# panuelosj/polystokes

Hardware: AMD Instinct MI355X
Metric: Stokes-solve wall ms/step (assembly+PCG) on 256^3 grid; CG iters/sec (lower is better)
Workload: dtype f64; 1 GPU; synthetic lid-driven cavity 256x256x256, reduced tiles (tile=16, pad=2), jacobi-PCG, tol 1e-3; parallelism=1 GPU

## Files before the change

polystokes_amd/__init__.py:

```python
import ctypes as C
import os
import subprocess

import numpy as np

from . import _abi
from ._abi import (FieldsIn, FieldsOut, Params, Scene, Stats, default_params)

_HERE = os.path.dirname(os.path.abspath(__file__))
LIB_PATH = os.environ.get("PS_LIB") or os.path.join(_HERE, "libpolystokes_hip.so")
_lib = None

EXPORTED_SYMBOLS = [
    "ps_abi_version", "ps_reduced_dof", "ps_context_create", "ps_context_destroy", "ps_last_error", "ps_params_default",
    "ps_upload_fields", "ps_step_device", "ps_setup_device", "ps_solve_device", "ps_download_fields",
    "polystokes_step", "ps_apply_operator", "ps_apply_preconditioner", "ps_query_array", "ps_read_array",
    "ps_export_component_matrices", "ps_export_matrices", "ps_export_stats", "ps_bench_kernel", "ps_memory_stats", "ps_set_interrupt", "ps_solve_exported_system",
    "ps_set_slab", "ps_set_brick", "ps_comm_unique_id", "ps_comm_init_rccl", "ps_comm_selftest", "ps_comm_init_tcp", "ps_dist_stats",
    "ps_group_create", "ps_group_destroy", "ps_group_rank", "ps_group_step",
    "ps_set_warm_start", "ps_download_solution_fields", "ps_upload_density_field", "ps_set_surface_tension",
    "ps_set_solid_boundary", "ps_set_rheology", "ps_set_solve_precision",
    "ps_upload_fields_device", "ps_upload_density_field_device", "ps_download_fields_device", "ps_download_solution_fields_device",
    "ps_step_device_fields", "ps_set_velocity_extrapolation",
]
# ... 162 lines not shown
    fi = FieldsIn()
    fi.nx, fi.ny, fi.nz = fields.nx, fields.ny, fields.nz
    fi.dx, fi.dt = fields.dx, fields.dt
    fi.orig[0] = fi.orig[1] = fi.orig[2] = 0.0
    fi.density = fields.density
    cv = getattr(fields, "collisionvel", None)
    for a in range(3):
        fi.vel[a] = device_address(fields.vel[a])
        fi.collisionvel[a] = device_address(cv[a]) if cv is not None else None
    fi.surface, fi.collision, fi.viscosity = (device_address(fields.surface), device_address(fields.collision),
                                              device_address(fields.viscosity))
    w = getattr(fields, "weights", None)
    for i in range(14):
        fi.weights[i] = device_address(w[i]) if w is not None else None
    return fi


_DT = {(1, "i"): np.int8, (4, "i"): np.int32, (4, "f"): np.float32, (8, "f"): np.float64, (4, "u"): np.uint32}


def _kind(name):
    if name.endswith(("Labels", "Indices", ".col", ".ptr", "Region", "Perm", ".chunkInfo", ".chunkRep", ".code")) or name.startswith("faceRow"):
        return "i"
    if name in ("valuesCoded", "columns16", "diagonalsCoded", "fusedStep", "streamRuns", "rowPerLane", "chebInner32", "warmStartUsed", "densityField", "launchWalk",
                "surfaceTensionReducedFaces", "solidBoundary", "solidSlipEdges", "rheologyModel", "rheologyIterations",
                "solvePrecisionUsed", "solvePassIterations",
                "velocityExtrapolation", "extrapolationLayerX", "extrapolationLayerY", "extrapolationLayerZ", "extrapolationCounts"):
        return "i"
    if name in ("ownedX", "ownedY", "ownedZ"):
        return "f"
    if False:
        return "i"
    if name == "reducedRowFace":
        return "u"
    return "f"


def process_memory_stats():
    v = (C.c_int64 * 4)()
    lib().ps_memory_stats(None, v)
    return {"live_bytes": int(v[0]), "peak_bytes": int(v[1]), "contexts": int(v[3])}


class PolyStokesError(RuntimeError):
    pass


# ... 392 lines not shown
```

polystokes_amd/csrc/ps_blocks.hip:

```cpp
#include "ps_context.hpp"
#include "ps_setup_util.hpp"

using namespace ps;

namespace {

constexpr int BS = SETUP_BS;

struct BlockArgs {
    Grid g;
    double invDx;
    const float* lw[7];
    const float* fw[7];
    const int32_t* lab[7];
    const int32_t* act[7];
    const int32_t* reg[7];
    const int32_t* sys[7];
    const int32_t* sysT[3];
    const int32_t* faceRow[3];
    const float* vel[3];
    const float* cvel[3];
    CellField visc;
    FaceDensity dens;
    int64_t nP, nA, faceOff[3];
// ... 922 lines not shown
            hipLaunchKernelGGL(k_St_edges<true>, dim3(gridFor(ne, BS)), dim3(BS), 0, stream, A, e, (int32_t*)nullptr, St.ptr.p, St.col.p,
                               v, St.code.p, rhsPT.p, uInv.p, wantExport ? uDiag.p : (double*)nullptr);
        }
    };
    {
        const int64_t n = g.count(0);
        hipLaunchKernelGGL(k_St_cells<false>, dim3(gridFor(n, BS)), dim3(BS), 0, stream, A, St.ptr.p, (const int32_t*)nullptr,
                           (int32_t*)nullptr, (double*)nullptr, (int8_t*)nullptr, (double*)nullptr, (double*)nullptr, (double*)nullptr);
        for (int e = 0; e < 3; ++e) {
            const int64_t ne = g.count(4 + e);
            hipLaunchKernelGGL(k_St_edges<false>, dim3(gridFor(ne, BS)), dim3(BS), 0, stream, A, e, St.ptr.p, (const int32_t*)nullptr,
                               (int32_t*)nullptr, (double*)nullptr, (int8_t*)nullptr, (double*)nullptr, (double*)nullptr, (double*)nullptr);
        }
        St.nnz = exclusiveScanI32(St.ptr.p, nSystem + 1);
        if (St.nnz != S.nnz) throw Error("internal: nnz(S^T) != nnz(S)");
        St.col.alloc((size_t)St.nnz); St.code.alloc((size_t)St.nnz);
        fillSt(forceFp64Values);
    }
    {
        const bool ok = readCounter(CTR_CODE_FAIL) == 0;
        if (!ok && !forceFp64Values) { fillS(true); fillSt(true); }
        S.packed = St.packed = ok && !forceFp64Values;
        valuesCodedHost = S.packed ? 1 : 0;
        buildDiagonalCodes();
        buildStreams(true);
        columns16Host = (S.col16ok ? 1 : 0) | (St.col16ok ? 2 : 0);
    }
}
```

polystokes_amd/csrc/ps_context.hip:

```cpp
#include <algorithm>
#include <chrono>
#include <cstdio>
#include <cstring>
#include <ctime>
#include <fstream>

#include "ps_context.hpp"
#include "ps_setup_util.hpp"

using namespace ps;

namespace {

struct StageTimer {
    hipEvent_t ev[PS_STAGE_COUNT + 1];
    hipStream_t s;
    int n = 0;
    explicit StageTimer(hipStream_t st) : s(st) {
        for (auto& e : ev) HIP_CHECK(hipEventCreate(&e));
    }
    ~StageTimer() { for (auto& e : ev) (void)hipEventDestroy(e); }
    void mark(int i) { HIP_CHECK(hipEventRecord(ev[i], s)); }
    double ms(int a, int b) { float f = 0; HIP_CHECK(hipEventElapsedTime(&f, ev[a], ev[b])); return f; }
};
// ... 195 lines not shown
        T.mark(1);
        classifyCells();
        if (P.doReducedRegions) constructReducedRegions(); else constructOnlyActiveRegions();
        setupPhaseDone = 0;
        return;
    }
    if (phase == 1) {
        classifyFaces();
        classifyEdges();
        T.mark(2);
        if (P.doReducedRegions) constructCenterReducedIndices(0);
        setupPhaseDone = 1;
        return;
    }
    if (P.doReducedRegions) {
        constructCenterReducedIndices(1);
        constructFacesReducedIndices();
        constructEdgesReducedIndices();
    }
    T.mark(3);
    constructActiveIndices();
    computeRheology();
    T.mark(4);
    if (P.doReducedRegions) {
        computeCenterOfMasses();
        computeLeastSquaresFits();
        computeReducedMassMatrices();
        computeReducedViscosityMatricesInteriorOnly();
    } else {
        fbItems = 0;
    }
    T.mark(5);
    constructMatrixBlocks();
    T.mark(6);
    assembleSystemPressureStressFactored();
    constructGuessVectors();
    T.mark(7);
    constructPreconditioner();
    T.mark(8);
    HIP_CHECK(hipStreamSynchronize(stream));
    const auto w1 = std::chrono::high_resolution_clock::now();
    std::memset(&lastStats, 0, sizeof(lastStats));
    lastStats.result = PS_INCOMPLETE;
    fillDimData(&lastStats);
    lastStats.solveData[0] = -1; lastStats.solveData[1] = -1; lastStats.solveData[2] = -1; lastStats.solveData[3] = -1;
    lastStats.solveData[4] = 1000.0 * (double)(std::clock() - Z.c0) / CLOCKS_PER_SEC;
    lastStats.solveData[5] = std::chrono::duration<double, std::milli>(w1 - Z.w0).count();
    lastStats.stage_ms[PS_STAGE_WEIGHTS] = T.ms(0, 1);
    lastStats.stage_ms[PS_STAGE_CLASSIFY] = T.ms(1, 2);
    lastStats.stage_ms[PS_STAGE_REGIONS] = T.ms(2, 3);
    lastStats.stage_ms[PS_STAGE_INDICES] = T.ms(3, 4);
    lastStats.stage_ms[PS_STAGE_TILE_MATRICES] = T.ms(4, 5);
    lastStats.stage_ms[PS_STAGE_BLOCKS] = T.ms(5, 6);
    lastStats.stage_ms[PS_STAGE_ASSEMBLE] = T.ms(6, 7);
    lastStats.stage_ms[PS_STAGE_PRECOND] = T.ms(7, 8);
    setupState.reset();
    setupPhaseDone = 2;
// ... 102 lines not shown
    regHost("solidBoundary", &solidBoundaryUsed, 1, 4);
    if (solidBoundaryUsed == PS_SOLID_FREE_SLIP) reg("solidSlipEdges", slipEdges.p, 1, 4);
    regHost("rheologyModel", &rheoModelUsed, 1, 4);
    if (rheoModelUsed != PS_RHEOLOGY_NEWTONIAN) {
        reg("rheologyStrainRate", rheoRate.p, g.count(0), 4);
        reg("rheologyViscosity", rheoMu.p, g.count(0), 4);
        regHost("rheologyIterations", rheoIters.data(), (int64_t)rheoIters.size(), 4);
    }
    regHost("velocityExtrapolation", &extrapUsedHost, 1, 4);
    if (extrapUsedHost > 0) {
        static const char* axn[3] = {"X", "Y", "Z"};
        for (int a = 0; a < 3; ++a) reg(std::string("extrapolationLayer") + axn[a], extrapLayer[a].p, g.count(1 + a), 1);
        reg("extrapolationCounts", extrapCounts.p, extrapUsedHost, 4);
    }
    if (P.preconditioner == PS_PRE_DIAGONAL) regp("dinv", dinv.p, nSystem, permSys.p, 0);
    if (isSolved) {
        regp("recoveredActiveVelocity", recovered.p, nActiveVs, permRow.p, 0);
        reg("recoveredReducedVelocity", recovered.p ? recovered.p + nActiveVs : nullptr, nReducedVs, 8);
    }
    regHost("valuesCoded", &valuesCodedHost, 1, 4);
    diagFlagsHost = (uCoded ? 1 : 0) | (mcCoded ? 2 : 0);
    regHost("diagonalsCoded", &diagFlagsHost, 1, 4);
    regHost("columns16", &columns16Host, 1, 4);
    regHost("fusedStep", &fusedStepHost, 1, 4);
    regHost("launchWalk", launchWalkHost, 5 * LAUNCH_WALK_FIELDS, 4);
    chebInner32Host = chebInner32 ? 1 : 0;
    regHost("chebInner32", &chebInner32Host, 1, 4);
    streamRunsHost[0] = S.col16ok ? (int32_t)S.uniqueLen : 0; streamRunsHost[1] = S.col16ok ? (int32_t)S.streamLen : 0;
    streamRunsHost[2] = St.col16ok ? (int32_t)St.uniqueLen : 0; streamRunsHost[3] = St.col16ok ? (int32_t)St.streamLen : 0;
    regHost("streamRuns", streamRunsHost, 4, 4);
    rowPerLaneHost[0] = ((S.ellok && S.packed) ? 1 : 0) | ((St.ellok && St.packed) ? 2 : 0); rowPerLaneHost[1] = ilPlaneMajor;
    regHost("rowPerLane", rowPerLaneHost, 2, 4);
    reg("sysPerm", permSys.p, nSystem, 4);
    reg("rowPerm", permRow.p, nActiveVs, 4);
    reg("S.ptr", S.ptr.p, S.rows + 1, 4); reg("S.col", S.col.p, S.nnz, 4); reg("S.val", S.val.p, S.nnz, 8);
    reg("St.ptr", St.ptr.p, St.rows + 1, 4); reg("St.col", St.col.p, St.nnz, 4); reg("St.val", St.val.p, St.nnz, 8);
    if (S.col16ok) { reg("S.chunkInfo", S.chunkInfo.p, (int64_t)S.nChunks * 4, 4); reg("S.chunkRep", S.chunkRep.p, S.nChunks, 4); }
    if (St.col16ok) { reg("St.chunkInfo", St.chunkInfo.p, (int64_t)St.nChunks * 4, 4); reg("St.chunkRep", St.chunkRep.p, St.nChunks, 4); }
    if (S.packed) reg("S.code", S.code.p, S.nnz, 1);
    if (St.packed) reg("St.code", St.code.p, St.nnz, 1);
    reg("reducedRowFace", rrowFace.p, nReducedRows, 4);
    reg("reducedRowRegion", rrowRegion.p, nReducedRows, 4);
    static const char* ax[3] = {"X", "Y", "Z"};
    for (int a = 0; a < 3; ++a) {
        reg(std::string("vel") + ax[a], velOut[a].p, g.count(1 + a), 4);
        reg(std::string("valid") + ax[a], valid[a].p, g.count(1 + a), 4);
// ... 138 lines not shown
int32_t ps_reduced_dof(void) { return PS_RD; }

ps_context* ps_context_create(int32_t device) {
    int count = 0;
    hipError_t e = hipGetDeviceCount(&count);
    if (e != hipSuccess || count <= 0) {
        g_createError = "polystokes: no HIP device available (the product path has no CPU fallback)";
        std::fprintf(stderr, "%s\n", g_createError.c_str());
        return nullptr;
    }
    if (device < 0 || device >= count) {
        g_createError = "polystokes: device index out of range";
        std::fprintf(stderr, "%s\n", g_createError.c_str());
        return nullptr;
    }
    ps_context* c = new ps_context();
    c->device = device;
    if (hipSetDevice(device) != hipSuccess || hipStreamCreateWithFlags(&c->stream, hipStreamNonBlocking) != hipSuccess) {
        delete c;
        g_createError = "polystokes: cannot initialise HIP device";
        std::fprintf(stderr, "%s\n", g_createError.c_str());
        return nullptr;
    }
    ps_params_default(&c->P);
    return c;
}

void ps_context_destroy(ps_context* c) {
    if (!c) return;
    (void)hipSetDevice(c->device);
    (void)hipStreamSynchronize(c->stream);
    ps_dist_release(c);
    hipStream_t s = c->ownsStream ? c->stream : nullptr;
    if (c->pinnedCounters) (void)hipHostFree(c->pinnedCounters);
    if (c->pinnedScan) (void)hipHostFree(c->pinnedScan);
    for (auto& e : c->fieldEv) if (e) (void)hipEventDestroy(e);
    delete c;
    ps::releaseDeferred(ps::orphanFrees());
    if (s) (void)hipStreamDestroy(s);
}

const char* ps_last_error(const ps_context* c) { return c ? c->err.c_str() : g_createError.c_str(); }

void ps_params_default(ps_params* p) {
    std::memset(p, 0, sizeof(*p));
    p->mindensity = 1; p->maxdensity = 100000;
    p->matrixSetup = PS_PRESSURE_STRESS; p->solverType = PS_PCG_MATRIX_VECTOR_PRODUCTS;
    p->doSolve = 1; p->keepNonConvergedResults = 1; p->useWarmStart = 1;
    p->tolerance = 1e-3; p->maxSolverIterations = 5000;
    p->useInputSurfaceWeights = 1; p->useInputCollisionWeights = 1;
    p->activeLiquidBoundaryLayerSize = 2; p->activeSolidBoundaryLayerSize = 2;
    p->doReducedRegions = 1; p->doTile = 1; p->tileSize = 16; p->tilePadding = 2;
    p->preconditioner = PS_PRE_IDENTITY; p->indexOrder = PS_ORDER_VOXEL_TILES; p->negateCollision = 1;
}

int32_t ps_upload_fields(ps_context* c, const ps_params* p, const ps_fields_in* in) {
    if (!c) return PS_FAILED;
    PS_TRY(c, { c->upload(p, in); return PS_SUCCESS; })
}
// ... 599 lines not shown
```

polystokes_amd/csrc/ps_context.hpp:

```cpp
#pragma once
#include <map>
#include <memory>

#include "ps_common.hpp"

namespace ps {

struct DevCSR {
    int64_t rows = 0, cols = 0, nnz = 0;
    DevBuf<int32_t> ptr;
    DevBuf<int32_t> col;
    DevBuf<double> val;
    DevBuf<int8_t> code;
    bool packed = false;
    DevBuf<uint16_t> col16;
    DevBuf<int8_t> code4;
    DevBuf<double> val4;
    DevBuf<int32_t> winBase;
    DevBuf<int4> chunkInfo;
    DevBuf<uint8_t> len8;
    DevBuf<int32_t> chunkRep;
    int nChunks = 0;
    int64_t uniqueLen = 0;
    bool col16ok = false;
    int nv = 2;
    int64_t streamLen = 0;
    DevBuf<uint16_t> ecol;
// ... 55 lines not shown
    void add(int32_t* ptr, int64_t len) { p[count] = ptr; n[count] = len; ++count; }
};

struct FieldTable {
    static constexpr int MAX = 23;
    const float* src[MAX]; float* dst[MAX];
    int32_t fast[MAX], mid[MAX], slow[MAX];
    int count = 0;
    void add(const float* s, float* d_, int3 d, bool srcZFastest) {
        src[count] = s; dst[count] = d_;
        fast[count] = srcZFastest ? d.z : d.x; mid[count] = d.y; slow[count] = srcZFastest ? d.x : d.z;
        ++count;
    }
    int64_t entries(int q) const { return (int64_t)fast[q] * mid[q] * slow[q]; }
};
void launchFieldsCopy(const FieldTable& T, hipStream_t s);
void launchFieldsSwapXZ(const FieldTable& T, hipStream_t s);
enum ScanWord { SCAN_BAD = 0, SCAN_DIFFERS = 1, SCAN_FIRST = 2, SCAN_WORDS = 3 };
void launchFieldScan(const float* f, int64_t n, bool nonFinite, uint32_t* out, hipStream_t s);

struct CellField;
struct FaceDensity;

}

struct ps_context {
    ps::DeferredFrees deferred;
    ps_context() { ps::MemState& M = ps::memState(); std::lock_guard<std::mutex> lk(M.m); M.lists.push_back(&deferred); ++M.contexts; }
    ~ps_context() {
        { ps::MemState& M = ps::memState(); std::lock_guard<std::mutex> lk(M.m); --M.contexts; for (size_t q = 0; q < M.lists.size(); ++q) if (M.lists[q] == &deferred) { M.lists.erase(M.lists.begin() + (long)q); break; } }
        ps::releaseDeferred(deferred);
    }
    ps_context(const ps_context&) = delete;
    ps_context& operator=(const ps_context&) = delete;
    void drainDeferred(bool streamIsIdle) {
        if (ps::threadedRanks()) return;
        if (!streamIsIdle && (!stream || hipStreamQuery(stream) != hipSuccess)) { (void)hipGetLastError(); return; }
        ps::releaseDeferred(deferred);
        ps::releaseDeferred(ps::orphanFrees());
    }
    int device = 0;
    hipStream_t stream = nullptr;
    std::string err;

    ps_params P{};
    ps::Grid g{0, 0, 0, 0};
    double dx = 0, invDx = 0, dt = 0, invDt = 0, rho = 0;
    double valScale = 0;
    bool forceFp64Values = false;
    bool haveInputWeights = false;
    bool viscUniform = false;
    float viscUniformValue = 0.f;
    double rhoScalar = 0, densMin = 0, densMax = 0;
    bool densField = false;
    int32_t densFieldHost = 0;
    bool uploaded = false, isSetup = false, isSolved = false;
    std::string uploadDensity(const float* field);
    hipEvent_t fieldEv[2] = {nullptr, nullptr};
    ps::DevBuf<uint32_t> fieldScan;
    uint32_t* pinnedScan = nullptr;
    ps::DevBuf<float> fieldScratch;
    void uploadCheck(const ps_params* p, const ps_fields_in* in) const;
    static const char* missingField(const ps_fields_in* in);
    void uploadReset(const ps_params* p, const ps_fields_in* in);
    void ingestHost(const ps_fields_in* in);
    void ingestDevice(const ps_fields_in* in, int layout, hipStream_t caller);
// ... 178 lines not shown

    int solveIterations = -1;
    double solveError = -1;
    int usedBiCGStab = 0;
    ps_stats lastStats{};

    std::map<std::string, ps::ArrayInfo> arrays;
    std::map<std::string, std::vector<char>> hostArrays;

    void upload(const ps_params* p, const ps_fields_in* in);
    void buildIntegrationWeightsAlt();
    void classifyCells();
    void constructReducedRegions();
    void constructOnlyActiveRegions();
    void classifyFaces();
    void classifyEdges();
    void constructCenterReducedIndices(int part);
    void constructFacesReducedIndices();
    void constructEdgesReducedIndices();
    void constructActiveIndices();
    void buildValidFaces();
    void computeRegionBoxes();
    void computeCenterOfMasses();
    void computeLeastSquaresFits();
    void computeReducedMassMatrices();
    void computeReducedViscosityMatricesInteriorOnly();
    void assembleReducedBlocks();
    void constructMatrixBlocks();
    void buildCol16(ps::DevCSR& M, ps::Counter failSlot, const std::vector<int32_t>& cuts, const uint8_t* rowCode, int codeRows);
    void buildEll(ps::DevCSR& M);
    void buildStreams(bool share);
    bool shareRuns = true;
    ps::DevBuf<int2> scrChunkRows; ps::DevBuf<int32_t> scrSlice, scrStart4, scrVals, scrKeep, scrRemap, scrEllCol, scrEllCode, scrEllW; ps::DevBuf<unsigned long long> scrHash, scrKeys, scrUniq;
    void ensureValues(ps::DevCSR& M);
    void buildVal4(ps::DevCSR& M);
    std::vector<int32_t> regionRowPtrHost;
    std::vector<int32_t> hostTab[20];
    void assembleSystemPressureStressFactored();
    void constructPreconditioner();
    int solve();
    void estimateLambdaMax();
    void applyPreconditionerDevice(const double* r, double* z, double* scratch);
    int chebyshevApply(const double* rvec, double* zA, double* zB, double* rzPartial, const ps::CGScalars* sc, bool firstDone = false, double** zOut = nullptr);
    double chebTheta() const;
    int ntLevel() const;
    int solveEigenCG();
    void constructGuessVectors();
    void buildExplicitA(std::vector<int64_t>& ptr, std::vector<int32_t>& col, std::vector<double>& val);
    void recoverVelocityFromPressureStress();
    void applySolutionToVelocity();
// ... 34 lines not shown
```

polystokes_amd/csrc/ps_kernels_cg.hpp:

```cpp
#pragma once

#ifndef PS_VEC_NT_X
#define PS_VEC_NT_X 1
#endif
#ifndef PS_VEC_NT_AP
#define PS_VEC_NT_AP 1
#endif
#ifndef PS_VEC_NT_R
#define PS_VEC_NT_R 1
#endif
#ifndef PS_VEC_NT_RX
#define PS_VEC_NT_RX 1
#endif
#ifndef PS_VEC_NT_P
#define PS_VEC_NT_P 0
#endif
#ifndef PS_VEC_NT_PL
#define PS_VEC_NT_PL 0
#endif
#ifndef PS_VEC_NT_U
#define PS_VEC_NT_U 1
#endif
#ifndef PS_VEC_NT_D
#define PS_VEC_NT_D 1
// ... 644 lines not shown
    for (int64_t i = (int64_t)blockIdx.x * blockDim.x + threadIdx.x; i < n; i += (int64_t)gridDim.x * blockDim.x) out[i] = a[i] * b[i];
}
__global__ void k_guess_finish(double* __restrict__ g, const double* __restrict__ uInv, const int32_t* __restrict__ permSys, int64_t nP, int64_t n) {
    for (int64_t i = (int64_t)blockIdx.x * blockDim.x + threadIdx.x; i < n; i += (int64_t)gridDim.x * blockDim.x) {
        if (i < nP) continue;
        const int32_t j = permSys[i];
        g[j] = -2. * uInv[j] * g[j];
    }
}
__global__ void k_lin(double* __restrict__ out, double ca, const double* __restrict__ a, double cb, const double* __restrict__ b, double cc,
                      const double* __restrict__ c, int64_t n) {
    for (int64_t i = (int64_t)blockIdx.x * blockDim.x + threadIdx.x; i < n; i += (int64_t)gridDim.x * blockDim.x) {
        double v = ca * a[i];
        if (b) v += cb * b[i];
        if (c) v += cc * c[i];
        out[i] = v;
    }
}

__global__ void __launch_bounds__(256) k_jacobi_diag(const int32_t* __restrict__ ptr, const int32_t* __restrict__ col, const double* __restrict__ val,
                              const int8_t* __restrict__ code, double valScale, int n, int nP,
                              int nA, double dt, const double* __restrict__ McInv, const double* __restrict__ uInv,
                              const uint32_t* __restrict__ rrowFace, const int32_t* __restrict__ rrowRegion, const double* __restrict__ COM,
                              double dx, int3 off, const double* __restrict__ Binv, double* __restrict__ dinv, int invert) {
    const int j = blockIdx.x * blockDim.x + threadIdx.x;
    const bool live = j < n;
    double diag = 0.;
    int p = live ? ptr[j] : 0;
    const int pe = live ? ptr[j + 1] : 0;
    while (true) {
        double q[PS_RD];
#pragma unroll
        for (int m = 0; m < PS_RD; ++m) q[m] = 0.;
        int cur = -1;
        while (p < pe) {
            const int f = col[p];
            const double v = val ? val[p] : (double)code[p] * valScale;
            if (f < nA) { diag += -dt * McInv[f] * v * v; ++p; continue; }
            const int rr = f - nA;
            const int r = rrowRegion[rr];
            if (cur >= 0 && r != cur) break;
            cur = r;
            double o[3];
            int axis;
            rowOffset(rrowFace[rr], COM, r, dx, off, o, &axis);
            double c[PS_RD];
            basisRow(o[0], o[1], o[2], axis, c);
// ... 1 lines not shown
            for (int m = 0; m < PS_RD; ++m) q[m] += c[m] * v;
            ++p;
        }
        bool pend = cur >= 0;
        unsigned long long todo = __ballot(pend);
        if (todo == 0ull) break;
        while (todo != 0ull) {
            const int rl = __builtin_amdgcn_readlane(cur, __ffsll((long long)todo) - 1);
            const double* __restrict__ B = Binv + (int64_t)rl * PS_RD * PS_RD;
            double s = 0.;
#pragma unroll
            for (int m = 0; m < PS_RD; ++m) {
                double t = 0.;
#pragma unroll
                for (int k = m + 1; k < PS_RD; ++k) t = __builtin_fma(B[m * PS_RD + k], q[k], t);
                s = __builtin_fma(q[m], __builtin_fma(B[m * PS_RD + m], q[m], 2. * t), s);
            }
            if (pend && cur == rl) { diag -= s; pend = false; }
            todo = __ballot(pend);
        }
    }
    if (!live) return;
    diag += -0.5 * uInv[j];
    dinv[j] = invert ? (diag != 0. ? 1. / diag : 1.) : diag;
}

__global__ void k_recover_active(const double* __restrict__ s, const double* __restrict__ McInv, const double* __restrict__ rhsA, double dt,
                                 double invDt, int64_t nA, double* __restrict__ ua) {
    for (int64_t f = (int64_t)blockIdx.x * blockDim.x + threadIdx.x; f < nA; f += (int64_t)gridDim.x * blockDim.x)
        ua[f] = dt * McInv[f] * (invDt * rhsA[f] - s[f]);
}
__global__ void k_writeback(Grid g, int axis, const int32_t* __restrict__ lab, const int32_t* __restrict__ act, const int32_t* __restrict__ reg,
                            const int32_t* __restrict__ faceRow, const double* __restrict__ ua, const double* __restrict__ creg, const double* __restrict__ COM,
                            double dx, int3 off, const float* __restrict__ cvel, const float* __restrict__ velIn, float* __restrict__ velOut, int apply) {
    const int3 d = g.dims(1 + axis);
    const int64_t c = (int64_t)blockIdx.x * blockDim.x + threadIdx.x;
    if (c >= (int64_t)d.x * d.y * d.z) return;
    const int l = lab[c];
    float out = velIn[c];
    if (apply && !(l == PS_UNSOLVED || l == PS_UNASSIGNED)) {
        const int r = reg[c];
        const int a = act[c];
        double v = 0.;
        if (r >= 0) {
            const int3 q = unlin3(d, c);
            double p[3] = {(double)(q.x + off.x), (double)(q.y + off.y), (double)(q.z + off.z)};
            p[axis] -= 0.5;
// ... 18 lines not shown
```

polystokes_amd/csrc/ps_solve.hip:

```cpp
#include <algorithm>
#include <chrono>
#include <iterator>
#include <cstring>
#include <cmath>
#include <limits>
#include <ctime>

#include "ps_context.hpp"

using namespace ps;

namespace {
#include "ps_kernels_spmv.hpp"
#include "ps_kernels_tiles.hpp"
#include "ps_kernels_cg.hpp"
}

namespace {
template <class F> auto withBool(bool b, F&& f) { if (b) f(std::true_type{}); else f(std::false_type{}); }
template <int V0, int... V, class F> auto withOneOf(int v, F&& f) {
    if constexpr (sizeof...(V) == 0) f(std::integral_constant<int, V0>{}); else if (v == V0) f(std::integral_constant<int, V0>{}); else withOneOf<V...>(v, f);
}
template <int V0, int... V, class F> auto withAtLeast(int v, F&& f) {
    if constexpr (sizeof...(V) == 0) f(std::integral_constant<int, V0>{}); else if (v >= V0) f(std::integral_constant<int, V0>{}); else withAtLeast<V...>(v, f);
// ... 384 lines not shown
        lin(w.x, 1., w.h, omega, w.s, 0., nullptr);
        const double xmag = std::sqrt(dot(w.x, w.x));
        apply(w.x, w.e);
        lin(w.e, 1., w.b, -1., w.e, 0., nullptr);
        const double rsnew = dot(w.e, w.e);
        rre = rsnew;
        if (std::sqrt(rsnew) / xmag < rre) rre = std::sqrt(rsnew) / xmag;
        if (rre < tol) { iters = i; break; }
        lin(w.r, 1., w.s, -omega, w.t, 0., nullptr);
    }
    err = rre;
    return iters;
}
}

void ps_context::applyOperator(const double* xdev, double* ydev, double* dotPartialsOut) {
    Launch L = mk(this, nullptr);
    L.spmvS(0, xdev, ts.p);
    L.tiles(0, ts.p);
    L.spmvSt(0, ts.p, xdev, nullptr, ydev, dotPartialsOut);
}

void ps_context::assembleSystemPressureStressFactored() {
    assembleReducedBlocks();
    applySurfaceTension();
    const int64_t n = nSystem;
    ts.alloc((size_t)nRows + 1);
    vreg.alloc((size_t)std::max<int64_t>(1, regionCount) * PS_RD);
    wreg.alloc((size_t)std::max<int64_t>(1, nRChunks) * PS_RD);
    b.alloc((size_t)n); x.alloc((size_t)n); r.alloc((size_t)n); pvec.alloc((size_t)n); Ap.alloc((size_t)n);
    dotPartials.alloc((size_t)std::max<int64_t>(3 * VGRID, gridFor(std::max<int64_t>(n, 1), BS)) + 16);
    scal.alloc(1);
    dotPartials2.alloc(RED_BLOCKS);
    dotPartials3.alloc(VGRID);
    dotPartialsR.alloc(2 * VGRID);
    if (nActiveVs > 0)
        hipLaunchKernelGGL(k_scale_rows, dim3(dotBlocks(nActiveVs)), dim3(BS), 0, stream, ts.p, McInv.p, rhsA.p, nActiveVs);
    Launch L = mk(this, nullptr);
    L.tiles(2, ts.p);
    L.spmvSt(1, ts.p, nullptr, rhsPT.p, b.p, nullptr);
    HIP_CHECK(hipMemsetAsync(x.p, 0, (size_t)std::max<int64_t>(n, 1) * sizeof(double), stream));
}

void ps_context::constructPreconditioner() {
    if (P.preconditioner != PS_PRE_DIAGONAL && P.preconditioner != PS_PRE_CHEBYSHEV && P.solverType != PS_EIGEN) return;
    dinv.alloc((size_t)nSystem);
    if (nSystem == 0) return;
    hipLaunchKernelGGL(k_jacobi_diag, dim3(gridFor(nSystem, 256)), dim3(256), 0, stream, St.ptr.p, St.col.p, (const double*)St.val.p, (const int8_t*)St.code.p, valScale, (int)nSystem,
                       (int)nPressures, (int)nActiveVs, dt, McInv.p, uInv.p, rrowFace.p, rrowRegion.p, COM.p, dx, make_int3(gOff[0], gOff[1], gOff[2]), Binv.p, dinv.p,
                       slabEnabled ? 0 : 1);
    dinvF.alloc((size_t)nSystem);
    if (!slabEnabled) hipLaunchKernelGGL(k_to_diag, dim3(dotBlocks(nSystem)), dim3(BS), 0, stream, dinv.p, dinvF.p, nSystem);
    if (P.preconditioner == PS_PRE_CHEBYSHEV && !slabEnabled) estimateLambdaMax();
}

int ps_context::ntLevel() const {
    static const int env = envInt(PS_ENV("PS_NT_LEVEL"), -1);
    if (env >= 0) return env;
    const int64_t rows = std::max(nSystem, deviceShareRows);
    return rows < NT_LEVEL1_MIN_ROWS ? 0 : (rows < NT_LEVEL2_MIN_ROWS ? 1 : 2);
}

double ps_context::chebTheta() const { return ChebRecurrence(chebLmax).theta; }

void ps_context::estimateLambdaMax() {
    const int64_t n = nSystem;
    chebLmax = 8.4;
    if (n == 0) return;
    const int vb = dotBlocks(n);
    tmp1.alloc((size_t)n); tmp2.alloc((size_t)n); tmp3.alloc((size_t)n);
    double* v = tmp1.p; double* w = tmp2.p; double* Av = tmp3.p;
    chebPartials.alloc((size_t)std::max<int64_t>(3 * VGRID, gridFor(n, BS)) + 16);
    hipLaunchKernelGGL(k_fill_f64, dim3(vb), dim3(BS), 0, stream, v, 1., n);
    chebLmax = powerLambdaMax([&] {
        applyOperator(v, Av, dotPartials.p);
// ... 520 lines not shown
```

polystokes_amd/csrc/ps_tiles.hip:

```cpp
#include "ps_context.hpp"
#include "ps_setup_util.hpp"

using namespace ps;

namespace {

constexpr int BS = SETUP_BS;
constexpr int FBATCH = 128;
constexpr int OUTW = PS_RD * PS_RD + PS_RD;

enum { MODE_MASS = 0, MODE_LSQ = 1, MODE_VISC = 2, MODE_MASS_FIELD = 3 };

struct TileArgs {
    Grid g;
    double dx;
    const int32_t* lab[7];
    const int32_t* reg[7];
    const float* vel[3];
    CellField visc;
    FaceDensity dens;
    const double* densFace[3];
    const double* COM;
    int3 off;
    const int32_t* bbox;
// ... 586 lines not shown
        double y[PS_RD];
        for (int i = 0; i < PS_RD; ++i) y[i] = (perm[i] == lane) ? 1. : 0.;
        for (int i = 0; i < PS_RD; ++i) { double s = y[i]; for (int j = 0; j < i; ++j) s -= lu[i][j] * y[j]; y[i] = s; }
        for (int i = PS_RD - 1; i >= 0; --i) { double s = y[i]; for (int j = i + 1; j < PS_RD; ++j) s -= lu[i][j] * y[j]; y[i] = s / lu[i][i]; }
        for (int i = 0; i < PS_RD; ++i) Binv[o + i * PS_RD + lane] = y[i];
    }
}

TileArgs makeArgs(ps_context* c) {
    TileArgs A;
    A.g = c->g; A.dx = c->dx;
    for (int s = 0; s < 7; ++s) { A.lab[s] = c->labels[s].p; A.reg[s] = c->reducedIdx[s].p; }
    for (int a = 0; a < 3; ++a) A.vel[a] = c->vel[a].p;
    A.visc = c->viscSource(); A.dens = c->densSource();
    for (int a = 0; a < 3; ++a) A.densFace[a] = c->densFace[a].p;
    A.COM = c->COM.p;
    A.off = make_int3(c->gOff[0], c->gOff[1], c->gOff[2]);
    A.bbox = c->bbox.p;
    A.itemRegion = c->fbItemRegion.p; A.itemAxis = c->fbItemAxis.p; A.itemStart = c->fbItemStart.p;
    return A;
}

template <int MODE>
void runOuter(ps_context* c, double* out676, double* out26) {
    if (c->regionCount == 0 || c->fbItems == 0) return;
    c->partials.alloc((size_t)c->fbItems * OUTW);
    TileArgs A = makeArgs(c);
    static const bool useMfma = envInt(PS_ENV("PS_TILE_VALU"), 0) == 0;
    static const int clsMask = envInt(PS_ENV("PS_TILE_CLASS_MASK"), 2);
    const bool shareable = MODE == MODE_VISC || (MODE == MODE_MASS && !c->densField);
    if (shareable && ((MODE == MODE_MASS ? 1 : 2) & clsMask) && c->tileReps > 0 && c->tileReps < c->regionCount) {
        A.itemRegion = c->repItemRegion.p; A.itemAxis = c->repItemAxis.p; A.itemStart = c->repItemStart.p;
        if (useMfma) hipLaunchKernelGGL(k_region_outer_mfma<MODE>, dim3((unsigned)c->repItems), dim3(BS), 0, c->stream, A, c->partials.p);
        else hipLaunchKernelGGL(k_region_outer<MODE>, dim3((unsigned)c->repItems), dim3(BS), 0, c->stream, A, c->partials.p);
        hipLaunchKernelGGL(k_region_sum_list, dim3((unsigned)c->tileReps), dim3(BS), 0, c->stream, c->partials.p, c->repRegionItemPtr.p, c->repList.p, out676);
        hipLaunchKernelGGL(k_tile_replicate, dim3((unsigned)c->regionCount), dim3(BS), 0, c->stream, (const int32_t*)c->tileRep.p, out676);
        return;
    }
    if (MODE == MODE_MASS && c->densField) {
        for (int a = 0; a < 3; ++a) {
            const int64_t n = c->g.count(1 + a);
            c->densFace[a].alloc((size_t)n);
            A.densFace[a] = c->densFace[a].p;
            hipLaunchKernelGGL(k_face_density, dim3(gridFor(n, BS)), dim3(BS), 0, c->stream, A, a, c->densFace[a].p);
        }
        if (useMfma) hipLaunchKernelGGL(k_region_outer_mfma<MODE_MASS_FIELD>, dim3((unsigned)c->fbItems), dim3(BS), 0, c->stream, A, c->partials.p);
        else hipLaunchKernelGGL(k_region_outer<MODE_MASS_FIELD>, dim3((unsigned)c->fbItems), dim3(BS), 0, c->stream, A, c->partials.p);
    } else if (useMfma) hipLaunchKernelGGL(k_region_outer_mfma<MODE>, dim3((unsigned)c->fbItems), dim3(BS), 0, c->stream, A, c->partials.p);
    else hipLaunchKernelGGL(k_region_outer<MODE>, dim3((unsigned)c->fbItems), dim3(BS), 0, c->stream, A, c->partials.p);
    hipLaunchKernelGGL(k_region_sum, dim3((unsigned)c->regionCount), dim3(BS), 0, c->stream, c->partials.p, c->fbRegionItemPtr.p, out676, out26);
}

}

void ps_context::computeCenterOfMasses() {
    computeRegionBoxes();
    const int64_t R = regionCount;
    COM.alloc((size_t)R * 3); cfit.alloc((size_t)R * PS_RD);
    Mr.alloc((size_t)R * PS_RD * PS_RD); Kv.alloc((size_t)R * PS_RD * PS_RD); Binv.alloc((size_t)R * PS_RD * PS_RD);
    rhsR.alloc((size_t)R * PS_RD);
    regionScratch.alloc((size_t)R * OUTW);
    if (R == 0) { fbItems = 0; return; }
    if (slabEnabled) {
        std::vector<int32_t> ro((size_t)R, 1);
        for (int64_t r = 0; r < R; ++r) {
            bool inside = true, outside = false;
            for (int a = 0; a < 3; ++a) {
                const int mn = hbbox[(size_t)r * 6 + a], mx = hbbox[(size_t)r * 6 + 3 + a];
                inside = inside && mn >= brick.lo[a] && mx < brick.hi[a];
                outside = outside || mx < brick.lo[a] || mn >= brick.hi[a];
            }
            if (!inside && !outside) throw Error("a reduced region straddles a cut of the decomposition (cuts must be tile aligned; doTile required)");
            ro[(size_t)r] = inside ? 1 : 0;
// ... 20 lines not shown
    fbItemRegion.alloc(iR.size()); fbItemAxis.alloc(iR.size()); fbItemStart.alloc(iR.size()); fbRegionItemPtr.alloc(ptr.size());
    {
        std::vector<int32_t>& sR = hostTab[4]; std::vector<int32_t>& sS = hostTab[5];
        sR.clear(); sS.clear();
        sbRegionItemPtrHost.assign((size_t)R + 1, 0);
        for (int64_t r = 0; r < R; ++r) {
            sbRegionItemPtrHost[(size_t)r] = (int32_t)sR.size();
            int64_t total = 1;
            for (int q = 0; q < 3; ++q) total *= (int64_t)hbbox[(size_t)r * 6 + 3 + q] - hbbox[(size_t)r * 6 + q] + 2;
            if (total > 0x7fffffff) throw Error("region face box too large");
            for (int64_t st = 0; st < total; st += FB_CHUNK) { sR.push_back((int32_t)r); sS.push_back((int32_t)st); }
        }
        sbRegionItemPtrHost[(size_t)R] = (int32_t)sR.size();
        sbItems = (int64_t)sR.size();
        sbItemRegion.alloc(sR.size()); sbItemStart.alloc(sS.size()); sbItemCount.alloc(sR.size() + 1);
        HIP_CHECK(hipMemcpyAsync(sbItemRegion.p, sR.data(), sR.size() * 4, hipMemcpyHostToDevice, stream));
        HIP_CHECK(hipMemcpyAsync(sbItemStart.p, sS.data(), sS.size() * 4, hipMemcpyHostToDevice, stream));
    }
    HIP_CHECK(hipMemcpyAsync(fbItemRegion.p, iR.data(), iR.size() * 4, hipMemcpyHostToDevice, stream));
    HIP_CHECK(hipMemcpyAsync(fbItemAxis.p, iA.data(), iA.size() * 4, hipMemcpyHostToDevice, stream));
    HIP_CHECK(hipMemcpyAsync(fbItemStart.p, iS.data(), iS.size() * 4, hipMemcpyHostToDevice, stream));
    HIP_CHECK(hipMemcpyAsync(fbRegionItemPtr.p, ptr.data(), ptr.size() * 4, hipMemcpyHostToDevice, stream));
    hipLaunchKernelGGL(k_com, dim3((unsigned)R), dim3(BS), 0, stream, g, dx, make_int3(gOff[0], gOff[1], gOff[2]), labels[0].p, reducedIdx[0].p, bbox.p, COM.p);
    buildTileClasses();
}

void ps_context::buildTileClasses() {
    tileReps = 0; repItems = 0;
    const int64_t R = regionCount;
    static const bool off = envInt(PS_ENV("PS_NO_TILE_CLASSES"), 0) != 0;
    if (off || R < 2) return;
    TileArgs A = makeArgs(this);
    unsigned cap = 1024;
    while (cap < 4u * (unsigned)R) cap <<= 1;
    tileSig.alloc((size_t)R * 2); tileUnique.alloc((size_t)R); tileRep.alloc((size_t)R);
    DevBuf<unsigned long long>& keys = scrKeys; DevBuf<int32_t>& vals = scrVals;
    keys.alloc(cap); vals.alloc(cap);
    HIP_CHECK(hipMemsetAsync(keys.p, 0xff, (size_t)cap * 8, stream));
    HIP_CHECK(hipMemsetAsync(vals.p, 0x7f, (size_t)cap * 4, stream));
    hipLaunchKernelGGL(k_tile_signature, dim3((unsigned)R), dim3(BS), 0, stream, A, tileSig.p, tileUnique.p);
    hipLaunchKernelGGL(k_tile_rep_insert, dim3(gridFor(R, BS)), dim3(BS), 0, stream, (const unsigned long long*)tileSig.p, (const int32_t*)tileUnique.p, (int)R, keys.p, vals.p, cap - 1);
    hipLaunchKernelGGL(k_tile_rep_verify, dim3((unsigned)R), dim3(BS), 0, stream, A, (const unsigned long long*)tileSig.p, (const int32_t*)tileUnique.p,
                       (const unsigned long long*)keys.p, (const int32_t*)vals.p, cap - 1, tileRep.p);
    std::vector<int32_t>& rep = hostTab[11];
    rep.assign((size_t)R, 0);
    HIP_CHECK(hipMemcpyAsync(rep.data(), tileRep.p, (size_t)R * 4, hipMemcpyDeviceToHost, stream));
// ... 5 lines not shown
        if (rep[(size_t)r] != (int32_t)r) continue;
        list.push_back((int32_t)r);
        ptr.push_back((int32_t)iR.size());
        for (int a = 0; a < 3; ++a) {
            int64_t e[3];
            for (int q = 0; q < 3; ++q) e[q] = (int64_t)hbbox[(size_t)r * 6 + 3 + q] - hbbox[(size_t)r * 6 + q] + 1;
            e[a] += 1;
            const int64_t total = e[0] * e[1] * e[2];
            for (int64_t st = 0; st < total; st += FB_CHUNK) { iR.push_back((int32_t)r); iA.push_back(a); iS.push_back((int32_t)st); }
        }
    }
    ptr.push_back((int32_t)iR.size());
    if ((int64_t)list.size() == R) return;
    tileReps = (int64_t)list.size(); repItems = (int64_t)iR.size();
    repItemRegion.alloc(iR.size()); repItemAxis.alloc(iA.size()); repItemStart.alloc(iS.size()); repRegionItemPtr.alloc(ptr.size()); repList.alloc(list.size());
    HIP_CHECK(hipMemcpyAsync(repItemRegion.p, iR.data(), iR.size() * 4, hipMemcpyHostToDevice, stream));
    HIP_CHECK(hipMemcpyAsync(repItemAxis.p, iA.data(), iA.size() * 4, hipMemcpyHostToDevice, stream));
    HIP_CHECK(hipMemcpyAsync(repItemStart.p, iS.data(), iS.size() * 4, hipMemcpyHostToDevice, stream));
    HIP_CHECK(hipMemcpyAsync(repRegionItemPtr.p, ptr.data(), ptr.size() * 4, hipMemcpyHostToDevice, stream));
    HIP_CHECK(hipMemcpyAsync(repList.p, list.data(), list.size() * 4, hipMemcpyHostToDevice, stream));
    if (PS_ENV_VERBOSE()) std::fprintf(stderr, "[polystokes] tile classes: %lld of %lld tiles sum their own Mr / K\n", (long long)tileReps, (long long)R);
}

void ps_context::computeLeastSquaresFits() {
    if (regionCount == 0) return;
    double* N = regionScratch.p;
    double* rhs = regionScratch.p + (size_t)regionCount * PS_RD * PS_RD;
    runOuter<MODE_LSQ>(this, N, rhs);
    hipLaunchKernelGGL(k_lsq_solve, dim3((unsigned)regionCount), dim3(64), 0, stream, N, rhs, cfit.p);
}
void ps_context::computeReducedMassMatrices() { runOuter<MODE_MASS>(this, Mr.p, nullptr); }
void ps_context::computeReducedViscosityMatricesInteriorOnly() { runOuter<MODE_VISC>(this, Kv.p, nullptr); }

void ps_context::assembleReducedBlocks() {
    if (regionCount == 0) return;
    hipLaunchKernelGGL(k_binv, dim3((unsigned)regionCount), dim3(64), 0, stream, invDt, Mr.p, Kv.p, cfit.p, Binv.p, rhsR.p);
}
```

Baseline: 994.3 ms/step.

## Overlap reduced-region tile assembly with matrix block construction on a side stream

```diff
diff --git a/polystokes_amd/__init__.py b/polystokes_amd/__init__.py
--- a/polystokes_amd/__init__.py
+++ b/polystokes_amd/__init__.py
@@ -208,7 +208,7 @@
 def _kind(name):
     if name.endswith(("Labels", "Indices", ".col", ".ptr", "Region", "Perm", ".chunkInfo", ".chunkRep", ".code")) or name.startswith("faceRow"):
         return "i"
-    if name in ("valuesCoded", "columns16", "diagonalsCoded", "fusedStep", "streamRuns", "rowPerLane", "chebInner32", "warmStartUsed", "densityField", "launchWalk",
+    if name in ("valuesCoded", "columns16", "diagonalsCoded", "fusedStep", "streamRuns", "rowPerLane", "setupOverlap", "chebInner32", "warmStartUsed", "densityField", "launchWalk",
                 "surfaceTensionReducedFaces", "solidBoundary", "solidSlipEdges", "rheologyModel", "rheologyIterations",
                 "solvePrecisionUsed", "solvePassIterations",
                 "velocityExtrapolation", "extrapolationLayerX", "extrapolationLayerY", "extrapolationLayerZ", "extrapolationCounts"):
diff --git a/polystokes_amd/csrc/ps_blocks.hip b/polystokes_amd/csrc/ps_blocks.hip
--- a/polystokes_amd/csrc/ps_blocks.hip
+++ b/polystokes_amd/csrc/ps_blocks.hip
@@ -968,6 +968,12 @@
         if (!ok && !forceFp64Values) { fillS(true); fillSt(true); }
         S.packed = St.packed = ok && !forceFp64Values;
         valuesCodedHost = S.packed ? 1 : 0;
+        if (setupMayFork(2) && (binvEarly || regionCount == 0) && jacobiWanted() && nSystem > 0) {
+            dinv.alloc((size_t)nSystem); dinvF.alloc((size_t)nSystem);
+            setupFJ.fork(2);
+            launchJacobiDiagonal(setupStream(), true);
+            jacobiEarly = true;
+        }
         buildDiagonalCodes();
         buildStreams(true);
         columns16Host = (S.col16ok ? 1 : 0) | (St.col16ok ? 2 : 0);
diff --git a/polystokes_amd/csrc/ps_context.hip b/polystokes_amd/csrc/ps_context.hip
--- a/polystokes_amd/csrc/ps_context.hip
+++ b/polystokes_amd/csrc/ps_context.hip
@@ -241,17 +241,26 @@
     constructActiveIndices();
     computeRheology();
     T.mark(4);
+    setupFJ.ops.main = stream;
+    ForkJoinScope<decltype(setupFJ)> forkScope(setupFJ);
+    setupOverlapHost = 0;
+    binvEarly = jacobiEarly = false;
     if (P.doReducedRegions) {
         computeCenterOfMasses();
-        computeLeastSquaresFits();
-        computeReducedMassMatrices();
-        computeReducedViscosityMatricesInteriorOnly();
+        hipStream_t ts = stream;
+        if (setupMayFork(1) && regionCount > 0) { setupFJ.fork(1); ts = setupStream(); }
+        computeLeastSquaresFits(ts);
+        computeReducedMassMatrices(ts);
+        computeReducedViscosityMatricesInteriorOnly(ts);
+        if (setupMayFork(3)) { assembleReducedBlocks(ts); binvEarly = true; }
     } else {
         fbItems = 0;
     }
     T.mark(5);
     constructMatrixBlocks();
     T.mark(6);
+    setupFJ.join();
+    setupOverlapHost = setupFJ.taken;
     assembleSystemPressureStressFactored();
     constructGuessVectors();
     T.mark(7);
@@ -400,6 +409,7 @@
     diagFlagsHost = (uCoded ? 1 : 0) | (mcCoded ? 2 : 0);
     regHost("diagonalsCoded", &diagFlagsHost, 1, 4);
     regHost("columns16", &columns16Host, 1, 4);
+    regHost("setupOverlap", &setupOverlapHost, 1, 4);
     regHost("fusedStep", &fusedStepHost, 1, 4);
     regHost("launchWalk", launchWalkHost, 5 * LAUNCH_WALK_FIELDS, 4);
     chebInner32Host = chebInner32 ? 1 : 0;
@@ -584,6 +594,15 @@
         std::fprintf(stderr, "%s\n", g_createError.c_str());
         return nullptr;
     }
+    {
+        static const int mask = envInt(PS_ENV("PS_SETUP_OVERLAP"), 3) & 3;
+        SetupStreamOps& o = c->setupFJ.ops;
+        o.main = c->stream;
+        if (mask != 0 && hipStreamCreateWithFlags(&o.side, hipStreamNonBlocking) == hipSuccess &&
+            hipEventCreateWithFlags(&o.ev[0], hipEventDisableTiming) == hipSuccess && hipEventCreateWithFlags(&o.ev[1], hipEventDisableTiming) == hipSuccess)
+            c->setupFJ.allowed = mask;
+        else (void)hipGetLastError();
+    }
     ps_params_default(&c->P);
     return c;
 }
@@ -597,6 +616,11 @@
     if (c->pinnedCounters) (void)hipHostFree(c->pinnedCounters);
     if (c->pinnedScan) (void)hipHostFree(c->pinnedScan);
     for (auto& e : c->fieldEv) if (e) (void)hipEventDestroy(e);
+    {
+        SetupStreamOps& o = c->setupFJ.ops;
+        if (o.side) { (void)hipStreamSynchronize(o.side); (void)hipStreamDestroy(o.side); }
+        for (auto& e : o.ev) if (e) (void)hipEventDestroy(e);
+    }
     delete c;
     ps::releaseDeferred(ps::orphanFrees());
     if (s) (void)hipStreamDestroy(s);
diff --git a/polystokes_amd/csrc/ps_context.hpp b/polystokes_amd/csrc/ps_context.hpp
--- a/polystokes_amd/csrc/ps_context.hpp
+++ b/polystokes_amd/csrc/ps_context.hpp
@@ -3,6 +3,7 @@
 #include <memory>
 
 #include "ps_common.hpp"
+#include "ps_fork_join.hpp"
 
 namespace ps {
 
@@ -104,6 +105,14 @@
 struct CellField;
 struct FaceDensity;
 
+struct SetupStreamOps {
+    hipStream_t main = nullptr, side = nullptr;
+    hipEvent_t ev[2] = {nullptr, nullptr};
+    void forkEdge() { HIP_CHECK(hipEventRecord(ev[0], main)); HIP_CHECK(hipStreamWaitEvent(side, ev[0], 0)); }
+    void joinEdge() { HIP_CHECK(hipEventRecord(ev[1], side)); HIP_CHECK(hipStreamWaitEvent(main, ev[1], 0)); }
+    void syncSide() noexcept { if (side && hipStreamSynchronize(side) != hipSuccess) (void)hipGetLastError(); }
+};
+
 }
 
 struct ps_context {
@@ -124,6 +133,13 @@
     int device = 0;
     hipStream_t stream = nullptr;
     std::string err;
+    ps::ForkJoin<ps::SetupStreamOps> setupFJ;
+    int32_t setupOverlapHost = 0;
+    bool binvEarly = false, jacobiEarly = false;
+    hipStream_t setupStream() const { return setupFJ.ops.side; }
+    bool setupMayFork(int bit) const { return setupFJ.may(bit) && !slabEnabled; }
+    void launchJacobiDiagonal(hipStream_t s, bool storeDiag);
+    bool jacobiWanted() const { return P.preconditioner == PS_PRE_DIAGONAL || P.preconditioner == PS_PRE_CHEBYSHEV || P.solverType == PS_EIGEN; }
 
     ps_params P{};
     ps::Grid g{0, 0, 0, 0};
@@ -348,10 +364,10 @@
     void buildValidFaces();
     void computeRegionBoxes();
     void computeCenterOfMasses();
-    void computeLeastSquaresFits();
-    void computeReducedMassMatrices();
-    void computeReducedViscosityMatricesInteriorOnly();
-    void assembleReducedBlocks();
+    void computeLeastSquaresFits(hipStream_t s);
+    void computeReducedMassMatrices(hipStream_t s);
+    void computeReducedViscosityMatricesInteriorOnly(hipStream_t s);
+    void assembleReducedBlocks(hipStream_t s);
     void constructMatrixBlocks();
     void buildCol16(ps::DevCSR& M, ps::Counter failSlot, const std::vector<int32_t>& cuts, const uint8_t* rowCode, int codeRows);
     void buildEll(ps::DevCSR& M);
diff --git a/polystokes_amd/csrc/ps_fork_join.hpp b/polystokes_amd/csrc/ps_fork_join.hpp
--- /dev/null
+++ b/polystokes_amd/csrc/ps_fork_join.hpp
@@ -0,0 +1,38 @@
+#pragma once
+
+namespace ps {
+
+template <class Ops>
+struct ForkJoin {
+    Ops ops{};
+    int allowed = 0;
+    int open = 0;
+    int taken = 0;
+    void begin() { open = 0; taken = 0; }
+    bool may(int bit) const { return (allowed & bit) != 0; }
+    void fork(int bit) {
+        ops.forkEdge();
+        open |= bit; taken |= bit;
+    }
+    void join() {
+        if (!open) return;
+        ops.joinEdge();
+        open = 0;
+    }
+    void abandon() noexcept {
+        if (!open) return;
+        open = 0;
+        ops.syncSide();
+    }
+};
+
+template <class FJ>
+struct ForkJoinScope {
+    FJ& f;
+    explicit ForkJoinScope(FJ& f_) : f(f_) { f.begin(); }
+    ~ForkJoinScope() { f.abandon(); }
+    ForkJoinScope(const ForkJoinScope&) = delete;
+    ForkJoinScope& operator=(const ForkJoinScope&) = delete;
+};
+
+}
diff --git a/polystokes_amd/csrc/ps_kernels_cg.hpp b/polystokes_amd/csrc/ps_kernels_cg.hpp
--- a/polystokes_amd/csrc/ps_kernels_cg.hpp
+++ b/polystokes_amd/csrc/ps_kernels_cg.hpp
@@ -690,7 +690,8 @@
                               const int8_t* __restrict__ code, double valScale, int n, int nP,
                               int nA, double dt, const double* __restrict__ McInv, const double* __restrict__ uInv,
                               const uint32_t* __restrict__ rrowFace, const int32_t* __restrict__ rrowRegion, const double* __restrict__ COM,
-                              double dx, int3 off, const double* __restrict__ Binv, double* __restrict__ dinv, int invert) {
+                              double dx, int3 off, const double* __restrict__ Binv, double* __restrict__ dinv, diag_t* __restrict__ dinvF,
+                              int invert) {
     const int j = blockIdx.x * blockDim.x + threadIdx.x;
     const bool live = j < n;
     double diag = 0.;
@@ -738,7 +739,9 @@
     }
     if (!live) return;
     diag += -0.5 * uInv[j];
-    dinv[j] = invert ? (diag != 0. ? 1. / diag : 1.) : diag;
+    const double d = invert ? (diag != 0. ? 1. / diag : 1.) : diag;
+    dinv[j] = d;
+    if (dinvF) dinvF[j] = diagStore(d);
 }
 
 __global__ void k_recover_active(const double* __restrict__ s, const double* __restrict__ McInv, const double* __restrict__ rhsA, double dt,
diff --git a/polystokes_amd/csrc/ps_solve.hip b/polystokes_amd/csrc/ps_solve.hip
--- a/polystokes_amd/csrc/ps_solve.hip
+++ b/polystokes_amd/csrc/ps_solve.hip
@@ -430,7 +430,7 @@
 }
 
 void ps_context::assembleSystemPressureStressFactored() {
-    assembleReducedBlocks();
+    if (!binvEarly) assembleReducedBlocks(stream);
     applySurfaceTension();
     const int64_t n = nSystem;
     ts.alloc((size_t)nRows + 1);
@@ -450,15 +450,20 @@
     HIP_CHECK(hipMemsetAsync(x.p, 0, (size_t)std::max<int64_t>(n, 1) * sizeof(double), stream));
 }
 
+void ps_context::launchJacobiDiagonal(hipStream_t s, bool storeDiag) {
+    hipLaunchKernelGGL(k_jacobi_diag, dim3(gridFor(nSystem, 256)), dim3(256), 0, s, St.ptr.p, St.col.p, (const double*)St.val.p, (const int8_t*)St.code.p, valScale, (int)nSystem,
+                       (int)nPressures, (int)nActiveVs, dt, McInv.p, uInv.p, rrowFace.p, rrowRegion.p, COM.p, dx, make_int3(gOff[0], gOff[1], gOff[2]), Binv.p, dinv.p,
+                       storeDiag ? dinvF.p : (diag_t*)nullptr, slabEnabled ? 0 : 1);
+}
 void ps_context::constructPreconditioner() {
-    if (P.preconditioner != PS_PRE_DIAGONAL && P.preconditioner != PS_PRE_CHEBYSHEV && P.solverType != PS_EIGEN) return;
-    dinv.alloc((size_t)nSystem);
-    if (nSystem == 0) return;
-    hipLaunchKernelGGL(k_jacobi_diag, dim3(gridFor(nSystem, 256)), dim3(256), 0, stream, St.ptr.p, St.col.p, (const double*)St.val.p, (const int8_t*)St.code.p, valScale, (int)nSystem,
-                       (int)nPressures, (int)nActiveVs, dt, McInv.p, uInv.p, rrowFace.p, rrowRegion.p, COM.p, dx, make_int3(gOff[0], gOff[1], gOff[2]), Binv.p, dinv.p,
-                       slabEnabled ? 0 : 1);
-    dinvF.alloc((size_t)nSystem);
-    if (!slabEnabled) hipLaunchKernelGGL(k_to_diag, dim3(dotBlocks(nSystem)), dim3(BS), 0, stream, dinv.p, dinvF.p, nSystem);
+    if (!jacobiWanted()) return;
+    if (!jacobiEarly) {
+        dinv.alloc((size_t)nSystem);
+        if (nSystem == 0) return;
+        launchJacobiDiagonal(stream, false);
+        dinvF.alloc((size_t)nSystem);
+        if (!slabEnabled) hipLaunchKernelGGL(k_to_diag, dim3(dotBlocks(nSystem)), dim3(BS), 0, stream, dinv.p, dinvF.p, nSystem);
+    }
     if (P.preconditioner == PS_PRE_CHEBYSHEV && !slabEnabled) estimateLambdaMax();
 }
 
diff --git a/polystokes_amd/csrc/ps_tiles.hip b/polystokes_amd/csrc/ps_tiles.hip
--- a/polystokes_amd/csrc/ps_tiles.hip
+++ b/polystokes_amd/csrc/ps_tiles.hip
@@ -632,33 +632,30 @@
 }
 
 template <int MODE>
-void runOuter(ps_context* c, double* out676, double* out26) {
+void runOuter(ps_context* c, double* out676, double* out26, hipStream_t s) {
     if (c->regionCount == 0 || c->fbItems == 0) return;
-    c->partials.alloc((size_t)c->fbItems * OUTW);
     TileArgs A = makeArgs(c);
     static const bool useMfma = envInt(PS_ENV("PS_TILE_VALU"), 0) == 0;
     static const int clsMask = envInt(PS_ENV("PS_TILE_CLASS_MASK"), 2);
     const bool shareable = MODE == MODE_VISC || (MODE == MODE_MASS && !c->densField);
     if (shareable && ((MODE == MODE_MASS ? 1 : 2) & clsMask) && c->tileReps > 0 && c->tileReps < c->regionCount) {
         A.itemRegion = c->repItemRegion.p; A.itemAxis = c->repItemAxis.p; A.itemStart = c->repItemStart.p;
-        if (useMfma) hipLaunchKernelGGL(k_region_outer_mfma<MODE>, dim3((unsigned)c->repItems), dim3(BS), 0, c->stream, A, c->partials.p);
-        else hipLaunchKernelGGL(k_region_outer<MODE>, dim3((unsigned)c->repItems), dim3(BS), 0, c->stream, A, c->partials.p);
-        hipLaunchKernelGGL(k_region_sum_list, dim3((unsigned)c->tileReps), dim3(BS), 0, c->stream, c->partials.p, c->repRegionItemPtr.p, c->repList.p, out676);
-        hipLaunchKernelGGL(k_tile_replicate, dim3((unsigned)c->regionCount), dim3(BS), 0, c->stream, (const int32_t*)c->tileRep.p, out676);
+        if (useMfma) hipLaunchKernelGGL(k_region_outer_mfma<MODE>, dim3((unsigned)c->repItems), dim3(BS), 0, s, A, c->partials.p);
+        else hipLaunchKernelGGL(k_region_outer<MODE>, dim3((unsigned)c->repItems), dim3(BS), 0, s, A, c->partials.p);
+        hipLaunchKernelGGL(k_region_sum_list, dim3((unsigned)c->tileReps), dim3(BS), 0, s, c->partials.p, c->repRegionItemPtr.p, c->repList.p, out676);
+        hipLaunchKernelGGL(k_tile_replicate, dim3((unsigned)c->regionCount), dim3(BS), 0, s, (const int32_t*)c->tileRep.p, out676);
         return;
     }
     if (MODE == MODE_MASS && c->densField) {
         for (int a = 0; a < 3; ++a) {
             const int64_t n = c->g.count(1 + a);
-            c->densFace[a].alloc((size_t)n);
-            A.densFace[a] = c->densFace[a].p;
-            hipLaunchKernelGGL(k_face_density, dim3(gridFor(n, BS)), dim3(BS), 0, c->stream, A, a, c->densFace[a].p);
-        }
-        if (useMfma) hipLaunchKernelGGL(k_region_outer_mfma<MODE_MASS_FIELD>, dim3((unsigned)c->fbItems), dim3(BS), 0, c->stream, A, c->partials.p);
-        else hipLaunchKernelGGL(k_region_outer<MODE_MASS_FIELD>, dim3((unsigned)c->fbItems), dim3(BS), 0, c->stream, A, c->partials.p);
-    } else if (useMfma) hipLaunchKernelGGL(k_region_outer_mfma<MODE>, dim3((unsigned)c->fbItems), dim3(BS), 0, c->stream, A, c->partials.p);
-    else hipLaunchKernelGGL(k_region_outer<MODE>, dim3((unsigned)c->fbItems), dim3(BS), 0, c->stream, A, c->partials.p);
-    hipLaunchKernelGGL(k_region_sum, dim3((unsigned)c->regionCount), dim3(BS), 0, c->stream, c->partials.p, c->fbRegionItemPtr.p, out676, out26);
+            hipLaunchKernelGGL(k_face_density, dim3(gridFor(n, BS)), dim3(BS), 0, s, A, a, c->densFace[a].p);
+        }
+        if (useMfma) hipLaunchKernelGGL(k_region_outer_mfma<MODE_MASS_FIELD>, dim3((unsigned)c->fbItems), dim3(BS), 0, s, A, c->partials.p);
+        else hipLaunchKernelGGL(k_region_outer<MODE_MASS_FIELD>, dim3((unsigned)c->fbItems), dim3(BS), 0, s, A, c->partials.p);
+    } else if (useMfma) hipLaunchKernelGGL(k_region_outer_mfma<MODE>, dim3((unsigned)c->fbItems), dim3(BS), 0, s, A, c->partials.p);
+    else hipLaunchKernelGGL(k_region_outer<MODE>, dim3((unsigned)c->fbItems), dim3(BS), 0, s, A, c->partials.p);
+    hipLaunchKernelGGL(k_region_sum, dim3((unsigned)c->regionCount), dim3(BS), 0, s, c->partials.p, c->fbRegionItemPtr.p, out676, out26);
 }
 
 }
@@ -725,6 +722,8 @@
     HIP_CHECK(hipMemcpyAsync(fbItemStart.p, iS.data(), iS.size() * 4, hipMemcpyHostToDevice, stream));
     HIP_CHECK(hipMemcpyAsync(fbRegionItemPtr.p, ptr.data(), ptr.size() * 4, hipMemcpyHostToDevice, stream));
     hipLaunchKernelGGL(k_com, dim3((unsigned)R), dim3(BS), 0, stream, g, dx, make_int3(gOff[0], gOff[1], gOff[2]), labels[0].p, reducedIdx[0].p, bbox.p, COM.p);
+    partials.alloc((size_t)fbItems * OUTW);
+    if (densField) for (int a = 0; a < 3; ++a) densFace[a].alloc((size_t)g.count(1 + a));
     buildTileClasses();
 }
 
@@ -776,17 +775,17 @@
     if (PS_ENV_VERBOSE()) std::fprintf(stderr, "[polystokes] tile classes: %lld of %lld tiles sum their own Mr / K\n", (long long)tileReps, (long long)R);
 }
 
-void ps_context::computeLeastSquaresFits() {
+void ps_context::computeLeastSquaresFits(hipStream_t s) {
     if (regionCount == 0) return;
     double* N = regionScratch.p;
     double* rhs = regionScratch.p + (size_t)regionCount * PS_RD * PS_RD;
-    runOuter<MODE_LSQ>(this, N, rhs);
-    hipLaunchKernelGGL(k_lsq_solve, dim3((unsigned)regionCount), dim3(64), 0, stream, N, rhs, cfit.p);
-}
-void ps_context::computeReducedMassMatrices() { runOuter<MODE_MASS>(this, Mr.p, nullptr); }
-void ps_context::computeReducedViscosityMatricesInteriorOnly() { runOuter<MODE_VISC>(this, Kv.p, nullptr); }
-
-void ps_context::assembleReducedBlocks() {
+    runOuter<MODE_LSQ>(this, N, rhs, s);
+    hipLaunchKernelGGL(k_lsq_solve, dim3((unsigned)regionCount), dim3(64), 0, s, N, rhs, cfit.p);
+}
+void ps_context::computeReducedMassMatrices(hipStream_t s) { runOuter<MODE_MASS>(this, Mr.p, nullptr, s); }
+void ps_context::computeReducedViscosityMatricesInteriorOnly(hipStream_t s) { runOuter<MODE_VISC>(this, Kv.p, nullptr, s); }
+
+void ps_context::assembleReducedBlocks(hipStream_t s) {
     if (regionCount == 0) return;
-    hipLaunchKernelGGL(k_binv, dim3((unsigned)regionCount), dim3(64), 0, stream, invDt, Mr.p, Kv.p, cfit.p, Binv.p, rhsR.p);
-}
+    hipLaunchKernelGGL(k_binv, dim3((unsigned)regionCount), dim3(64), 0, s, invDt, Mr.p, Kv.p, cfit.p, Binv.p, rhsR.p);
+}
```

After: 1002 ms/step (median of 2 runs). Within noise of the previous version (+0.7%).
